# ml-unito/PartitionedLS.jl

Measured on AMD Instinct MI355X. Metric: sign-pattern NNLS solves/sec (whole node); fp64 obj gap vs ref, higher is better.
Workload: dtype f64

## Files before the change

### partitionedls.jl_amd/csrc/opt.hip

```cpp
#include "ctx.h"
#include "near_tie.h"
#include "sweep_rules.h"
#include <algorithm>
#include <chrono>
#include <cmath>
#include <cstdio>
#include <cstring>
#include <functional>
#include <thread>

namespace partls {

static bool opt_range_ok(const partls_ctx *c, const char *who)
{
    if (c->kbits <= 40) return true;
    set_error("%s: %d sign bits: the enumeration of 2^(K+1) patterns is out of range (K <= 39); fit(Alt) and fit(BnB) take up to 61 groups", who, c->kbits);
    return false;
}

static void cleanup_opt(const partls_ctx *c, const std::vector<double> &w, uint64_t pattern, double *alpha, double *beta, double *t)
{
    const int64_t M = c->M, K = c->K;
    std::vector<double> a((size_t)M, 0.0);
    for (int64_t m = 0; m < M; ++m) {
        const int f = sign_of_var(c->mask_aug[(size_t)m], pattern);
        a[(size_t)m] = (f != 0) ? w[(size_t)m] / (double)f : 0.0;
        if (a[(size_t)m] < 0.0) a[(size_t)m] = 0.0;
    }
    std::vector<double> A((size_t)K, 0.0);
    for (int64_t k = 0; k < K; ++k) {
        double s = 0.0;
        for (int64_t m = 0; m < M; ++m) s += (double)c->P[(size_t)m + (size_t)k * M] * a[(size_t)m];
        const double sk = ((pattern >> k) & 1ULL) ? 1.0 : -1.0;
        beta[k] = sk * s;
        A[(size_t)k] = (s == 0.0) ? 1.0 : s;
    }
    for (int64_t m = 0; m < M; ++m) {
        double s = 0.0;
        for (int64_t k = 0; k < K; ++k) s += (double)c->P[(size_t)m + (size_t)k * M] * a[(size_t)m] / A[(size_t)k];
        alpha[m] = s;
    }
    *t = w[(size_t)M];
}

}

using namespace partls;

extern "C" {

partls_status partls_opt_prepare(partls_ctx *c, const double *X, int64_t N, int64_t M, int64_t ldX, const double *y,
                                 int x_on_device, const int64_t *P, int64_t K, int64_t ldP, double eta, uint32_t flags)
try {
    return ctx_prepare(c, X, N, M, ldX, y, x_on_device, P, K, ldP, eta, (flags & PARTLS_OPT_FAITHFUL_INTERCEPT) != 0, flags);
}
PARTLS_ABI_GUARD

partls_status partls_opt_prepare_weighted(partls_ctx *c, const double *X, int64_t N, int64_t M, int64_t ldX, const double *y,
                                          const double *w, int x_on_device, const int64_t *P, int64_t K, int64_t ldP, double eta,
                                          uint32_t flags)
try {
    return ctx_prepare(c, X, N, M, ldX, y, x_on_device, P, K, ldP, eta, (flags & PARTLS_OPT_FAITHFUL_INTERCEPT) != 0, flags, w);
}
PARTLS_ABI_GUARD

partls_status partls_opt_prepare_f32(partls_ctx *c, const float *X, int64_t N, int64_t M, int64_t ldX, const double *y, const double *w,
                                     int x_on_device, const int64_t *P, int64_t K, int64_t ldP, double eta, uint32_t flags)
try {
    return ctx_prepare(c, X, N, M, ldX, y, x_on_device, P, K, ldP, eta, (flags & PARTLS_OPT_FAITHFUL_INTERCEPT) != 0, flags, w, true);
}
PARTLS_ABI_GUARD

partls_status partls_opt_prepare_csr(partls_ctx *c, const int64_t *indptr, const int32_t *indices, const double *values, int64_t N, int64_t M,
                                     const double *y, const double *w, int x_on_device, const int64_t *P, int64_t K, int64_t ldP, double eta,
                                     uint32_t flags)
try {
    return ctx_prepare_csr(c, indptr, indices, values, N, M, y, w, x_on_device, P, K, ldP, eta, (flags & PARTLS_OPT_FAITHFUL_INTERCEPT) != 0, flags);
}
PARTLS_ABI_GUARD

int64_t partls_opt_num_patterns(const partls_ctx *c) { return (c && c->prepared && c->kbits <= 40) ? ((int64_t)1 << c->kbits) : 0; }

static partls_status sweep_second_pass(partls_ctx *c, int64_t g_begin, int64_t g_end, double *all_opt, double *bobj_io, int64_t *bpat_io,
                                       unsigned long long *unconv_io);

partls_status partls_opt_sweep(partls_ctx *c, int64_t g_begin, int64_t g_end, double *best_obj, int64_t *best_pattern,
                               double *all_opt, int64_t *n_unconverged)
try {
    if (!c || !c->prepared) { set_error("partls_opt_sweep: context not prepared"); return PARTLS_ERR_STATE; }
    if (!opt_range_ok(c, "partls_opt_sweep")) return PARTLS_ERR_UNSUPPORTED;
    const int64_t npat = (int64_t)1 << c->kbits;
    if (g_end < 0) g_end = npat;
    if (g_begin < 0 || g_begin > g_end || g_end > npat) { set_error("bad Gray-index range [%lld,%lld)", (long long)g_begin, (long long)g_end); return PARTLS_ERR_BAD_ARG; }
    if (all_opt && !c->faithful) { set_error("all_opt needs PARTLS_OPT_FAITHFUL_INTERCEPT"); return PARTLS_ERR_BAD_ARG; }
    PARTLS_HIP_CHECK(hipSetDevice(c->device));
    if (g_begin == g_end) {
        if (best_obj) *best_obj = INFINITY;
        if (best_pattern) *best_pattern = -1;
        if (n_unconverged) *n_unconverged = 0;
        return PARTLS_OK;
    }
    if (!c->order_ready) {
        partls_status st = prepare_sweep_order(c);
        if (st != PARTLS_OK) return st;
    }
    const int n = c->n;
    const int64_t total = g_end - g_begin;
    int64_t chain_len = 0;
    int grid = 0;
    if (!sweep_plan(c, total, &chain_len, &grid, "partls_opt_sweep")) return PARTLS_ERR_UNSUPPORTED;

    const size_t sweep_words = sweep_block_words(grid, true);
    PARTLS_HIP_CHECK(c->bestObj.ensure(sizeof(double) * sweep_block_words(std::max(grid, 4096), true)));
    PARTLS_HIP_CHECK(hipMemsetAsync(c->bestObj.p, 0, 4 * sizeof(unsigned long long), c->stream));
    if (all_opt) {
        PARTLS_HIP_CHECK(c->allOpt.ensure((size_t)npat * sizeof(double)));
        if (total < npat) PARTLS_HIP_CHECK(hipMemsetAsync(c->allOpt.p, 0xFF, (size_t)npat * sizeof(double), c->stream));
    }
    const partls_status ss = ensure_sweep_scratch(c, grid);
    if (ss != PARTLS_OK) return ss;

    SweepParams p = sweep_params(c, true);
    p.g_begin = g_begin; p.g_end = g_end; p.chain_len = chain_len;
    p.pair = sweep_pairs(c, total) ? 1 : 0;
    p.all_opt = all_opt ? c->allOpt.as<double>() : nullptr;
    bind_sweep_block(p, c->bestObj.as<double>(), grid, true);
    if (!c->use_reg && c->knobs.lz_fault) p.coop_fault = 77;
    c->export_wg = -1;
    if (((c->use_reg && (sweep_reg_small(c->T) || sweep_reg_exports(c->T))) || (!c->use_reg && !c->knobs.eager_generic)) && !c->knobs.no_export) {
        PARTLS_HIP_CHECK(c->bestSol.ensure((size_t)grid * n * sizeof(double)));
        p.best_sol = c->bestSol.as<double>();
        p.node_ld = n;
    }

    t_begin(c, PARTLS_T_SWEEP);
    PARTLS_HIP_CHECK(launch_any_sweep(c, p, grid));
    t_end(c, PARTLS_T_SWEEP);

    unsigned long long cnt[3] = {0, 0, 0};
    PARTLS_HIP_CHECK(c->sweepOut.resize(sweep_words));
    const double *sweep_out = c->sweepOut.data();
    PARTLS_HIP_CHECK(hipMemcpyAsync(c->sweepOut.data(), c->bestObj.p, sweep_words * sizeof(double), hipMemcpyDeviceToHost, c->stream));
    if (all_opt) {
        const void *src = c->allOpt.p;
        if (!c->order_identity) {
            PARTLS_HIP_CHECK(c->allOptRef.ensure((size_t)npat * sizeof(double)));
            PARTLS_HIP_CHECK(launch_pattern_gather(c->allOpt.as<double>(), npat, c->kbits, c->order, c->allOptRef.as<double>(), c->stream));
            src = c->allOptRef.p;
        }
        PARTLS_HIP_CHECK(hipMemcpyAsync(all_opt, src, (size_t)npat * sizeof(double), hipMemcpyDeviceToHost, c->stream));
    }
    PARTLS_HIP_CHECK(hipStreamSynchronize(c->stream));
    t_collect(c);
    std::memcpy(cnt, sweep_out, sizeof(cnt));
    if (c->knobs.print_stamps) {
        double st[32] = {0};
        if (hipMemcpy(st, c->scratch.p, sizeof(st), hipMemcpyDeviceToHost) == hipSuccess)
            fprintf(stderr, "[partls stamps] scan: pre %.0f barrier %.0f post %.0f | gather: work %.0f barrier %.0f | panel: work %.0f barrier %.0f | "
                            "update %.0f | scatter %.0f | chain-load %.0f/%.0f | pivots %llu || gather split: block setup %.0f chain %.0f rhs/myj %.0f"
                            " || workgroup 0: %.0f blocks, %.0f scans, %.0f pivots || pair walk: twin scan %.0f, solve + rows + scan %.0f\n",
                    st[9], st[10], st[0], st[12] + st[13] + st[8], st[1], st[11], st[2], st[3], st[4], st[5], st[6], cnt[1], st[12], st[13], st[8],
                    st[24], st[25], st[26], st[15], st[14]);
    }
    double bobj = INFINITY;
    int64_t bpat = -1;
    install_sweep_result(c, sweep_out, grid, p.best_sol != nullptr, &bobj, &bpat);
    if (rescue_on(c)) {
        rescue_begin_call(c);
        if (cnt[0]) {
            const partls_status rs = sweep_second_pass(c, g_begin, g_end, all_opt, &bobj, &bpat, &cnt[0]);
            if (rs != PARTLS_OK) return rs;
        }
    }
    if (best_obj) *best_obj = bobj;
    if (best_pattern) *best_pattern = bpat;
    if (n_unconverged) *n_unconverged = (int64_t)cnt[0];
    return PARTLS_OK;
}
PARTLS_ABI_GUARD

partls_status partls_opt_finish(partls_ctx *c, int64_t pattern, double *alpha, double *beta, double *t, double *opt,
                                int64_t *best_index)
try {
    if (!c || !c->prepared) { set_error("partls_opt_finish: context not prepared"); return PARTLS_ERR_STATE; }
    if (!alpha || !beta || !t || !opt) { set_error("partls_opt_finish: NULL output"); return PARTLS_ERR_BAD_ARG; }
    if (pattern < 0 || pattern >= ((int64_t)1 << (c->K + 1))) { set_error("pattern out of range"); return PARTLS_ERR_BAD_ARG; }
    PARTLS_HIP_CHECK(hipSetDevice(c->device));
    const uint64_t kmask = ((uint64_t)1 << c->kbits) - 1;
    uint64_t used = 1ULL << c->K;
    for (int i = 0; i < c->n; ++i) if (c->hScale[(size_t)i] != 0.0) used |= c->mask_tab[(size_t)i];

    std::vector<uint64_t> cands{(uint64_t)pattern & kmask & used};
    if (pattern == c->near_for)
        for (int64_t q : c->near_pat) {
            const uint64_t v = (uint64_t)q & kmask & used;
            if (std::find(cands.begin(), cands.end(), v) == cands.end()) cands.push_back(v);
        }
    const int export_wg = (pattern == c->near_for) ? c->export_wg : -1;
    c->export_wg = -1;
    c->near_for = -1;
    c->near_pat.clear();
    c->last_near_evaluated = (int64_t)cands.size();

    t_begin(c, PARTLS_T_FINISH);
    const auto f0 = std::chrono::steady_clock::now();
    std::vector<double> sols, obj2, w, wbest, g, gbest;
    std::vector<int8_t> codes;
    unsigned long long unconv = 0, unconv_best = 0;
    double obest = INFINITY, loo_best = 0.0;
    uint64_t pbest = cands[0];
    for (size_t ci = 0; ci < cands.size(); ++ci) {
        partls_status st = PARTLS_OK;
        bool taken = false;
        if (ci == 0 && export_wg >= 0) {
            PARTLS_HIP_CHECK(c->exportSol.resize((size_t)c->n));
            PARTLS_HIP_CHECK(hipMemcpyAsync(c->exportSol.data(), c->bestSol.as<double>() + (size_t)export_wg * c->n, (size_t)c->n * sizeof(double), hipMemcpyDeviceToHost, c->stream));
            PARTLS_HIP_CHECK(hipStreamSynchronize(c->stream));
            sols.assign(c->exportSol.data(), c->exportSol.data() + c->n);
            opt_codes(c, cands[ci], codes);
            taken = true;
            double smax = 0.0;
            for (int i = 0; i < c->n; ++i) smax = std::max(smax, std::fabs(sols[(size_t)i]));
            for (int i = 0; i < c->n && taken; ++i) {
                const double v = sols[(size_t)i];
                if (!std::isfinite(v)) taken = false;
                else if (v != 0.0 && (codes[(size_t)i] == 0 || (codes[(size_t)i] == 1 && v < -1e-9 * smax) || (codes[(size_t)i] == -1 && v > 1e-9 * smax))) taken = false;
            }
            if (taken) { c->tab_valid = false; unconv = 0; }
            if (c->knobs.finish_trace) fprintf(stderr, "[finish] the sweep's solution of its winner (workgroup %d): %s\n", export_wg, taken ? "taken" : "refused (signs), solving again");
        }
        if (!taken) {
            opt_codes(c, cands[ci], codes);
            st = solve_nodes(c, codes, 1, sols, obj2, &unconv, false, true);
            if (st != PARTLS_OK) return st;
            if (unconv && rescue_on(c)) {
                st = rescue_pattern(c, cands[ci], sols, nullptr, &unconv);
                if (st != PARTLS_OK) return st;
                c->tab_valid = false;
            }
        }
        unscale_solution(c, sols.data(), w);
        RefineOut ro;
        st = refine_solution(c, w, !c->faithful, 2, &ro);
        if (st != PARTLS_OK) return st;
        double o = 0.0;
        if (ro.have) { o = ro.obj; g.swap(ro.g); }
        else { st = data_objective(c, w, &o, &g); if (st != PARTLS_OK) return st; }
        if (c->knobs.finish_trace && cands.size() > 1) fprintf(stderr, "[finish] near tie: pattern %llu data objective %.17g\n", (unsigned long long)cands[ci], o);
        if (ci == 0 || o < obest || (o == obest && cands[ci] < pbest)) { obest = o; pbest = cands[ci]; wbest = w; gbest = g; unconv_best = unconv; loo_best = c->last_min_loo; }
    }
    const auto f1 = std::chrono::steady_clock::now();
    uint64_t full = pbest;
    if (!c->faithful) { if (wbest[(size_t)c->M] > 0.0) full |= (1ULL << c->K); }
    full &= used;
    std::vector<int8_t> vcode((size_t)c->M + 1, 0);
    for (int64_t m = 0; m <= c->M; ++m) {
        if (m == c->M && !c->faithful) { vcode[(size_t)m] = 2; continue; }
        const int f = sign_of_var(c->mask_aug[(size_t)m], full);
        vcode[(size_t)m] = (int8_t)((f > 0) - (f < 0));
    }
    int worst = -1;
    c->last_kkt = kkt_violation_data(c, wbest, gbest, vcode, &worst);
    *opt = obest;
    if (c->knobs.finish_trace) {
        const auto f2 = std::chrono::steady_clock::now();
        auto ms = [](auto a, auto b) { return std::chrono::duration<double, std::milli>(b - a).count(); };
        fprintf(stderr, "[finish] %zu candidate(s): solve + refine + data objective / gradient %.3f ms, KKT check %.3f ms; data-space KKT violation %.3e (variable %d)\n",
                cands.size(), ms(f0, f1), ms(f1, f2), c->last_kkt, worst);
    }
    t_end(c, PARTLS_T_FINISH);
    PARTLS_HIP_CHECK(hipStreamSynchronize(c->stream));
    t_collect(c);
    cleanup_opt(c, wbest, full, alpha, beta, t);
    if (best_index) *best_index = (int64_t)full;
    if (unconv_best) { set_error("winner re-solve hit the pivot cap"); return PARTLS_ERR_NOT_CONVERGED; }
    c->last_min_loo = loo_best;
    if (kkt_says_ill_conditioned(c)) {
        set_error("the winner's KKT conditions do not hold in data space (violation %.2e of ||x|| ||y|| at variable %d, tolerance %.1e; %llu columns "
                  "refused as dependent in the sweep): X is too ill-conditioned for the fp64 Gram form (cond(X) >~ 1e6); the outputs hold the best "
                  "Gram-form model", c->last_kkt, worst, c->knobs.kkt_tol, c->sweep_vetoes);
        return PARTLS_ERR_ILL_CONDITIONED;
    }
    return PARTLS_OK;
}
PARTLS_ABI_GUARD

partls_status partls_opt_pattern(partls_ctx *c, int64_t pattern, double *raw_alpha, double *optval)
try {
    if (!c || !c->prepared) { set_error("partls_opt_pattern: context not prepared"); return PARTLS_ERR_STATE; }
    if (!c->faithful) { set_error("partls_opt_pattern needs a context prepared with PARTLS_OPT_FAITHFUL_INTERCEPT"); return PARTLS_ERR_STATE; }
    if (pattern < 0 || pattern >= ((int64_t)1 << c->kbits)) { set_error("pattern out of range"); return PARTLS_ERR_BAD_ARG; }
    PARTLS_HIP_CHECK(hipSetDevice(c->device));
    std::vector<double> sols, obj2, w;
    unsigned long long unconv = 0;
    std::vector<int8_t> codes;
    opt_codes(c, (uint64_t)pattern, codes);
    partls_status st = solve_nodes(c, codes, 1, sols, obj2, &unconv, false, true);
    if (st != PARTLS_OK) return st;
    if (unconv && rescue_on(c)) {
        st = rescue_pattern(c, (uint64_t)pattern, sols, nullptr, &unconv);
        if (st != PARTLS_OK) return st;
        c->tab_valid = false;
    }
    unscale_solution(c, sols.data(), w);
    st = refine_solution(c, w, false);
    if (st != PARTLS_OK) return st;
    if (optval) { st = data_objective(c, w, optval); if (st != PARTLS_OK) return st; }
    if (raw_alpha)
        for (int64_t m = 0; m <= c->M; ++m) {
            const int f = sign_of_var(c->mask_aug[(size_t)m], (uint64_t)pattern);
            const double a = (f != 0) ? w[(size_t)m] / (double)f : 0.0;
            raw_alpha[m] = a > 0.0 ? a : 0.0;
        }
    if (unconv) { set_error("pattern solve hit the pivot cap"); return PARTLS_ERR_NOT_CONVERGED; }
    return PARTLS_OK;
// ... 437 lines not shown
```

### partitionedls.jl_amd/csrc/sweep_blk.hip

```cpp
#include "sweep_rules.h"
#include <atomic>
#include <type_traits>

namespace partls {
namespace blk {

static constexpr int THREADS = 512;
static constexpr int MAXT = 20;
#ifndef PARTLS_UPD_UNROLL
#define PARTLS_UPD_UNROLL 1
#endif
static constexpr int MB = 8;
#ifndef PARTLS_EXPORT_BIG
#define PARTLS_EXPORT_BIG 1
#endif
#ifndef PARTLS_MERGED_SCAN
#define PARTLS_MERGED_SCAN 1
#endif
#ifndef PARTLS_LANE_MASKS
#define PARTLS_LANE_MASKS 1
#endif
#ifndef PARTLS_MB_BIG
#define PARTLS_MB_BIG 8
#endif
#ifndef PARTLS_PAIR
#define PARTLS_PAIR 1
#endif
static constexpr int EXPORT_MAXT = 17;
static constexpr int MBB = PARTLS_MB_BIG;
static constexpr int NO_VETO = 99;
static constexpr int PAIR_MAXC = 16;
static constexpr int PAIR_PIV_MIN_HI = 0x3f1a36e2;
static constexpr int F64_EXP_HI = 0x7ff00000;

constexpr int nslots(int T) { return T * (T + 1) / 2; }
constexpr int tri(int g) { return g * (g + 1) / 2; }
constexpr int split(int T)
{
    int best = 1, bestmax = 1 << 30;
    for (int g = 1; g < T; ++g) {
        int a = tri(g), b = nslots(T) - tri(g);
        int m = a > b ? a : b;
        if (m < bestmax) { bestmax = m; best = g; }
    }
    return T == 1 ? 1 : best;
}
constexpr int rstride(int T) { return (T % 2) ? T : T + 1; }
constexpr int colw(int T) { return 513; }
static constexpr int MAXT_S = 10;
static constexpr int CW_S = 257;
template <class PT> __device__ __forceinline__ PT *uniform_ptr(PT *p)
{
    const unsigned long long v = (unsigned long long)p;
    const unsigned lo = (unsigned)__builtin_amdgcn_readfirstlane((int)v), hi = (unsigned)__builtin_amdgcn_readfirstlane((int)(v >> 32));
    return (PT *)(((unsigned long long)hi << 32) | lo);
}

#ifdef PARTLS_STAMPS
#define STAMP_DECL unsigned long long st_acc[24] = {0, 0, 0, 0, 0, 0, 0, 0, 0, 0, 0, 0, 0, 0, 0, 0, 0, 0, 0, 0, 0, 0, 0, 0}; unsigned long long st_t = __builtin_amdgcn_s_memtime();
#define STAMP(ph) do { __builtin_amdgcn_sched_barrier(0); unsigned long long _n = __builtin_amdgcn_s_memtime(); \
                       st_acc[ph] += _n - st_t; st_t = _n; __builtin_amdgcn_sched_barrier(0); } while (0)
#ifndef PARTLS_STAMP_TID
#define PARTLS_STAMP_TID 0
#endif
#define STAMP_FLUSH do { if (tid == PARTLS_STAMP_TID && blockIdx.x == 0 && p.scratch) { for (int _i = 0; _i < 24; ++_i) p.scratch[_i] = (double)st_acc[_i]; \
                                p.scratch[24] = (double)bc; p.scratch[25] = (double)sc; p.scratch[26] = (double)npiv; } } while (0)
#else
#define STAMP_DECL
#define STAMP(ph) do { } while (0)
#define STAMP_FLUSH do { } while (0)
#endif

static constexpr int CWMAX = colw(MAXT);
template <int CWX, int MAXTX>
struct LdsImageT {
    double Z[MB * CWX];
    double U[2 * (MB + 64)];
    double Dinv[MB + 64];
    unsigned long long s_inf[32];
    unsigned long long s_bas[16];
    unsigned long long s_sum[16];
    int s_veto[2];
    double s_best[4];
    unsigned char s_rbit[64];
    unsigned long long s_vmask[16 * MAXTX];
    double Pbase[2 * MB * CWX];
};
struct LdsImage {
    double Z[MBB * CWMAX];
    double U[2 * (MBB + 64)];
    double Dinv[MBB + 64];
    unsigned long long s_inf[32];
    unsigned long long s_bas[16];
    unsigned long long s_sum[16];
    int s_veto[2];
    double s_best[4];
    unsigned char s_rbit[64];
    unsigned long long s_vmask[16 * MAXT];
    double Pbase[2 * MBB * CWMAX];
};
static_assert(2 * MBB >= PAIR_MAXC, "the pair walk gathers up to PAIR_MAXC columns into the two panel buffers");
__shared__ LdsImage lds_image;
__shared__ LdsImageT<CW_S, MAXT_S> lds_small;

template <int W>
__device__ __forceinline__ auto *image_of()
{
    if constexpr (W == 1) return &lds_small; else return &lds_image;
}

template <int T, int H, int W = 2>
struct Half {
    static constexpr int G = W == 1 ? T : split(T);
    static constexpr int GLO = H ? G : 0;
    static constexpr int GHI = H ? T : G;
    static constexpr int OFF = H ? tri(G) : 0;
    static constexpr int CNT = (H ? nslots(T) - tri(G) : tri(G)) > 0 ? (H ? nslots(T) - tri(G) : tri(G)) : 1;
    static constexpr int XN = GHI;
    static constexpr int RS = rstride(T);
    static constexpr int CW = W == 1 ? CW_S : colw(T);
    static constexpr int NT = W == 1 ? 256 : THREADS;
    __device__ static constexpr int idx(int rho, int gam) { return tri(gam) + rho - OFF; }
};

template <class L>
__device__ __forceinline__ void tiles_store(double *dst, const double (&S)[L::CNT], int t8)
{
    double *bp = uniform_ptr(dst) + (size_t)L::OFF * 256;
#pragma unroll
    for (int s = 0; s < L::CNT; ++s) {
        if ((s & 1) == 0) asm volatile("" : "+s"(bp));
        bp[(s & 1) * 256 + t8] = S[s];
        if (s & 1) bp += 512;
    }
}

template <int T, int H, int W, int KAPPA, class SA>
__device__ __forceinline__ void gather_tile(const SA &S, double *P, int a, int b, unsigned pm)
{
    using L = Half<T, H, W>;
    if constexpr (KAPPA >= L::GLO && KAPPA < L::GHI) {
        if ((pm >> b) & 1u) {
            double *col = P + __builtin_popcount(pm & ((1u << b) - 1u)) * L::CW + a * L::RS;
#pragma unroll
            for (int rho = 0; rho <= KAPPA; ++rho) col[rho] = S[L::idx(rho, KAPPA)];
        }
    }
    if ((pm >> a) & 1u) {
        double *col = P + __builtin_popcount(pm & ((1u << a) - 1u)) * L::CW + b * L::RS;
#pragma unroll
        for (int gam = (KAPPA + 1 > L::GLO ? KAPPA + 1 : L::GLO); gam < L::GHI; ++gam) col[gam] = S[L::idx(KAPPA, gam)];
    }
}

template <int T, int H, int W, int KAPPA, class SA>
__device__ __forceinline__ void scatter_tile(SA &S, const double *P, int a, int b, unsigned pm)
{
    using L = Half<T, H, W>;
    if constexpr (KAPPA >= L::GLO && KAPPA < L::GHI) {
        if ((pm >> b) & 1u) {
            const double *col = P + __builtin_popcount(pm & ((1u << b) - 1u)) * L::CW + a * L::RS;
#pragma unroll
            for (int rho = 0; rho <= KAPPA; ++rho) S[L::idx(rho, KAPPA)] = col[rho];
        }
    }
    if ((pm >> a) & 1u) {
        const double *col = P + __builtin_popcount(pm & ((1u << a) - 1u)) * L::CW + b * L::RS;
#pragma unroll
        for (int gam = (KAPPA > L::GLO ? KAPPA : L::GLO); gam < L::GHI; ++gam) S[L::idx(KAPPA, gam)] = col[gam];
    }
}

template <int M, int CW, int MBK>
__device__ __forceinline__ int panel_block(double *P, double *Z, double *U, double *Dinv, int myj, bool my_basic,
                                           double piv_eps, int tid, int prow, bool idle_wave)
{
    if (idle_wave) {
#pragma unroll
        for (int s = 0; s < M; ++s) __syncthreads();
        return M;
    }
    constexpr int US = MBK + 64;
    const int dummy = MBK + (tid & 63);
    double pv[M];
#pragma unroll
    for (int j = 0; j < M; ++j) pv[j] = P[j * CW + prow];
    const int uslot = myj >= 0 ? myj : dummy;
    int veto = M;
#pragma unroll
    for (int s = 0; s < M; ++s) {
        Z[s * CW + prow] = pv[s];
        U[(s & 1) * US + uslot] = pv[s];
        if (myj == s) {
            const double d = pv[s];
            Dinv[s] = (my_basic || d > piv_eps) ? rcp_newton(d) : 0.0;
        }
        __syncthreads();
        double inv = Dinv[s];
        double u[M];
#pragma unroll
        for (int j = 0; j < M; ++j) u[j] = U[(s & 1) * US + j];
        asm volatile("" : "+v"(inv));
#pragma unroll
        for (int j = 0; j < M; ++j) asm volatile("" : "+v"(u[j]));
        if ((pv[s] * pv[s]) * (inv * piv_eps) >= 1.0) veto = veto < s ? veto : s;
        if (__builtin_amdgcn_readfirstlane(__double2hiint(inv)) & 0x7ff00000) {
            const double ainv = fabs(inv), fz = -pv[s] * inv;
            if (myj == s) {
#pragma unroll
                for (int j = 0; j < M; ++j) pv[j] = (j == s) ? -inv : u[j] * ainv;
            } else {
#pragma unroll
                for (int j = 0; j < M; ++j) pv[j] = (j == s) ? pv[s] * ainv : fma(fz, u[j], pv[j]);
            }
        }
    }
#pragma unroll
    for (int j = 0; j < M; ++j) P[j * CW + prow] = pv[j];
    return veto;
}

template <int CW, int RS, int KC>
__device__ __forceinline__ void pair_solve(const double *P, const int *cpos, int m, int lane, int rhspos, double *out)
{
    const int r = lane & 15, h = lane >> 4;
    const int code = cpos[r < m ? r : 0];
    const unsigned basm = (unsigned)__ballot(code < 0 && lane < m);
    const int kr = code < 0 ? ~code : code;
    const int pos = kr * RS + KC;
    double pv[4];
#pragma unroll
    for (int jj = 0; jj < 4; ++jj) {
        const int c = 4 * h + jj;
        const int cc = cpos[c < m ? c : 0];
        const double v = P[(cc < 0 ? ~cc : cc) * CW + pos];
        pv[jj] = (r < m && c < m) ? v : 0.0;
    }
    double qc = P[kr * CW + rhspos];
    if (r >= m) qc = 0.0;
    bool hard = false;
#pragma unroll 1
    for (int s = 0; s < m; ++s) {
        const double d = readlane_f64(pv[0], s);
        const int dh = __double2hiint(d);
        if ((!((basm >> s) & 1u) && !(dh > PAIR_PIV_MIN_HI)) || (dh & F64_EXP_HI) == F64_EXP_HI) { hard = true; break; }
        const double inv = rcp_newton(d), ainv = fabs(inv);
        const double pvs = __shfl(pv[0], r);
        const double fz = -pvs * inv;
        const double qs = readlane_f64(qc, s);
        double val[4];
#pragma unroll
        for (int jj = 0; jj < 4; ++jj) {
            const double u = __shfl(pv[0], (s + 4 * h + jj) & 15);
            val[jj] = (r == s) ? u * ainv : fma(fz, u, pv[jj]);
        }
        if (h == 0) val[0] = (r == s) ? -inv : pvs * ainv;
        qc = (r == s) ? qs * ainv : fma(fz, qs, qc);
        const double nx = __shfl(val[0], (lane + 16) & 63);
        pv[0] = val[1]; pv[1] = val[2]; pv[2] = val[3]; pv[3] = nx;
    }
    if (lane < PAIR_MAXC) {
        out[PAIR_MAXC + lane] = qc;
        out[lane] = ((basm >> lane) & 1u) ? -qc : qc;
    }
    if (lane == 0) out[2 * PAIR_MAXC + 1] = hard ? 1.0 : 0.0;
}

#define PARTLS_CASES(M) M(0) M(1) M(2) M(3) M(4) M(5) M(6) M(7) M(8) M(9) M(10) M(11) M(12) M(13) M(14) M(15) M(16) M(17) M(18) M(19)

template <int T, int H, bool NODE, int W = 2, bool MODELS = false, bool BATCH = false, bool PAIRK = false>
__device__ __forceinline__ void sweep_body(const SweepParams &p)
{
    using L = Half<T, H, W>;
    constexpr int RS = L::RS, CW = L::CW, RHSPOS = 16 * RS, NW = (T + 3) / 4;
    constexpr int THREADS = L::NT;
    constexpr int MB = W == 1 ? blk::MB : MBB;
    static_assert(!(NODE && MODELS), "node mode exports no per-pattern models (finish_pattern's capped flag is chain mode's)");
    constexpr bool MERGED = PARTLS_MERGED_SCAN && !NODE && !BATCH && T <= 17;
    constexpr bool LANE_MASKS = PARTLS_LANE_MASKS && !BATCH && T <= 16;
    constexpr bool PAIR = PAIRK && PARTLS_PAIR && MERGED && LANE_MASKS && W == 2 && !MODELS;
    static_assert(PAIR == PAIRK, "the pair walk is launched only where it is compiled (pair_compiled)");
    static_assert(W == 2 || RHSPOS < 256, "the 256-thread kernel needs every panel row position (and the rhs row) below 256");
    auto &lds_image = *image_of<W>();
    const int tid = threadIdx.x, t8 = tid & 255, a = t8 & 15, b = t8 >> 4, lane = tid & 63, wave = tid >> 6;
    const int n = p.n;
    const int nwords = (n + 63) >> 6;

    double *const Pbase = lds_image.Pbase, *const Z = lds_image.Z, *const U = lds_image.U, *const Dinv = lds_image.Dinv;
    unsigned long long *const s_inf = lds_image.s_inf, *const s_bas = lds_image.s_bas, *const s_vmask = lds_image.s_vmask;
    unsigned long long *const s_sum = lds_image.s_sum;
    int *const s_veto = lds_image.s_veto;
    double *const s_best = lds_image.s_best;
    [[maybe_unused]] double *const s_pair = U;
    [[maybe_unused]] int *const s_cpos = reinterpret_cast<int *>(Dinv);
    [[maybe_unused]] int *const s_tw = s_cpos + PAIR_MAXC;
    [[maybe_unused]] int *const s_cm = s_tw + 8;
    static_assert(2 * (MB + 64) >= 2 * PAIR_MAXC + 2, "pair_solve's `out` (doubles) fits U");
    static_assert(2 * (MB + 64) >= PAIR_MAXC + 9, "s_cpos, s_tw and s_cm (PAIR_MAXC + 9 ints) fit Dinv (MB + 64 doubles)");
    for (int i = tid; i < 2 * MB * CW; i += THREADS) Pbase[i] = 0.0;
    for (int i = tid; i < MB * CW; i += THREADS) Z[i] = 0.0;
    if (tid < 2 * (MB + 64)) U[tid] = 0.0;
    if (tid < MB + 64) Dinv[tid] = 0.0;
    if (tid < 32) s_inf[tid] = 0;
    if (tid < 16) { s_bas[tid] = 0; s_sum[tid] = 0; }
    if (tid < 2) s_veto[tid] = NO_VETO;
    if (tid == 0) {
        s_best[0] = __builtin_inf(); reinterpret_cast<long long *>(s_best)[1] = -1;
        s_best[2] = __builtin_inf(); reinterpret_cast<long long *>(s_best)[3] = -1;
    }
    if (tid < 16 * T) s_vmask[tid] = tid < p.n ? p.mask[tid] : 0ULL;
    if (tid < 64) lds_image.s_rbit[tid] = tid < 40 ? p.rbit.gbit[tid] : 0;
    __syncthreads();

    double S[L::CNT];
    double q = 0.0, corner = 0.0;
    double mybest = __builtin_inf();
    const bool has_var = tid < n;
    bool basic = false, blocked = false;
    const int mypos = (tid & 15) * RS + (tid >> 4);
    const int rowc = tid / RS, rowrho = tid - rowc * RS;
    const bool idle_wave = __builtin_amdgcn_readfirstlane((tid & ~63) > RHSPOS ? 1 : 0) != 0;

    unsigned npiv = 0, nunconv = 0, nveto = 0;
    unsigned bc = 0, sc = 0;

    const int clen = (int)p.chain_len;
    const int nchains = (int)((p.g_end - p.g_begin + clen - 1) / clen);

    STAMP_DECL
    for (int chain = blockIdx.x; chain < nchains; chain += gridDim.x) {
        const int64_t g0 = p.g_begin + (int64_t)chain * clen;
        const int glen = (int)((g0 + clen < p.g_end) ? clen : p.g_end - g0);
        STAMP(5);
        const double *src = p.T0;
        if constexpr (NODE) {
            if (p.node_src) {
                const double *snap = p.node_src[chain];
                if (snap) src = snap;
            }
        }
        {
            const double *bp = uniform_ptr(src) + (size_t)L::OFF * 256;
#pragma unroll
            for (int s = 0; s < L::CNT; ++s) {
                if ((s & 1) == 0) asm volatile("" : "+s"(bp));
                S[s] = bp[(s & 1) * 256 + t8];
                if (s & 1) bp += 512;
            }
        }
        q = (tid < 16 * T) ? src[(size_t)nslots(T) * 256 + tid] : 0.0;
        corner = src[(size_t)nslots(T) * 256 + 16 * T];
        basic = false;
        if constexpr (NODE) {
            if (src != p.T0 && tid < 16 * T) basic = reinterpret_cast<const int8_t *>(src + (nslots(T) * 256 + 16 * T + 8))[tid] != 0;
        }
        STAMP(6);

        auto finish_pattern = [&](int gi, [[maybe_unused]] bool capped) {
            const uint64_t g = (uint64_t)g0 + (unsigned)gi;
            const uint64_t pat = NODE ? (uint64_t)chain : g ^ (g >> 1);
            const double obj2 = corner > 0.0 ? corner : 0.0;
            if constexpr (NODE) {
                if (p.node_piv && tid == 0) {
                    unsigned *o = p.node_piv + 3 * ((size_t)chain * clen + gi);
                    o[0] = npiv; o[1] = bc; o[2] = sc;
                }
            }
            if (p.all_opt && tid == THREADS - 1) p.all_opt[pat] = sqrt(obj2);
            if constexpr (MODELS) {
                const size_t row = (size_t)chain * (size_t)clen + (size_t)gi;
                if (has_var) p.node_sol[row * p.node_ld + tid] = capped ? __builtin_nan("") : (basic ? q : 0.0);
                if (tid == THREADS - 1) p.node_obj2[row] = capped ? __builtin_nan("") : sqrt(obj2);
            }
            if constexpr (!NODE && !MODELS && (W == 1 || (PARTLS_EXPORT_BIG && T <= EXPORT_MAXT))) {
                if (p.best_sol && obj2 < mybest) {
                    mybest = obj2;
                    if (has_var) p.best_sol[(size_t)blockIdx.x * p.node_ld + tid] = basic ? q : 0.0;
                }
            }
            if (tid == THREADS - 1 && obj2 <= s_best[2]) {
                const double bo = s_best[0];
                const long long bp = reinterpret_cast<long long *>(s_best)[1];
                if (obj2 < bo || (obj2 == bo && ref_index_less(pat, (unsigned long long)bp, lds_image.s_rbit))) {
                    s_best[2] = bo; reinterpret_cast<long long *>(s_best)[3] = bp;
                    s_best[0] = obj2; reinterpret_cast<long long *>(s_best)[1] = (long long)pat;
                } else if (obj2 < s_best[2] || ref_index_less(pat, (unsigned long long)reinterpret_cast<long long *>(s_best)[3], lds_image.s_rbit)) {
                    s_best[2] = obj2; reinterpret_cast<long long *>(s_best)[3] = (long long)pat;
                }
            }
        };
        [[maybe_unused]] auto record_twin = [&](int gi, double cornerv, double qv, bool bv) {
            const uint64_t g = (uint64_t)g0 + (unsigned)gi;
            const uint64_t pat = g ^ (g >> 1);
            const double obj2 = cornerv > 0.0 ? cornerv : 0.0;
            if (p.all_opt && tid == THREADS - 1) p.all_opt[pat] = sqrt(obj2);
            if constexpr (PARTLS_EXPORT_BIG && T <= EXPORT_MAXT) {
                if (p.best_sol && obj2 < mybest) {
                    mybest = obj2;
                    if (has_var) p.best_sol[(size_t)blockIdx.x * p.node_ld + tid] = bv ? qv : 0.0;
                }
            }
            if (tid == THREADS - 1 && obj2 <= s_best[2]) {
                const double bo = s_best[0];
                const long long bp = reinterpret_cast<long long *>(s_best)[1];
                if (obj2 < bo || (obj2 == bo && ref_index_less(pat, (unsigned long long)bp, lds_image.s_rbit))) {
                    s_best[2] = bo; reinterpret_cast<long long *>(s_best)[3] = bp;
                    s_best[0] = obj2; reinterpret_cast<long long *>(s_best)[1] = (long long)pat;
                } else if (obj2 < s_best[2] || ref_index_less(pat, (unsigned long long)reinterpret_cast<long long *>(s_best)[3], lds_image.s_rbit)) {
                    s_best[2] = obj2; reinterpret_cast<long long *>(s_best)[3] = (long long)pat;
                }
            }
        };
        int gi = 0;
        [[maybe_unused]] bool tw_pending = false;
        [[maybe_unused]] auto pair_partner = [&](int i) -> int {
            const int j = (((unsigned)g0 + (unsigned)i) & 1u) ? i - 1 : i + 1;
            return (PAIR && j >= 0 && j < glen) ? j : -1;
        };
        [[maybe_unused]] auto pair_unit_end = [&](int i) -> int { const int j = pair_partner(i); return (j > i ? j : i) + 1; };
        [[maybe_unused]] auto pair_target = [&](int u, int i) -> int {
            const unsigned gu = (unsigned)g0 + (unsigned)u, gc = (unsigned)g0 + (unsigned)i;
            if (pair_partner(u) < 0 || (gu & 1u)) return u;
            return (((gu >> 1) ^ gu ^ (gc >> 1) ^ gc) & 1u) ? u + 1 : u;
        };
        [[maybe_unused]] auto pair_next = [&](bool to_twin, int &f, int &fn) -> bool {
            if (to_twin) gi = pair_partner(gi);
            else {
                const int u = pair_unit_end(gi);
                if (u >= glen) return false;
                gi = pair_target(u, gi);
            }
            tw_pending = !to_twin && pair_partner(gi) >= 0;
            const uint64_t vmask = s_vmask[tid < 16 * T ? tid : 0] & (has_var ? ~0ULL : 0ULL);
            const uint64_t g = (uint64_t)g0 + (unsigned)gi;
            f = sign_of_var(vmask, g ^ (g >> 1));
            const int u2 = pair_unit_end(gi);
            fn = f;
            if (u2 < glen) { const uint64_t gn = (uint64_t)g0 + (unsigned)pair_target(u2, gi); fn = sign_of_var(vmask, gn ^ (gn >> 1)); }
            return true;
        };
        for (;;) {
            [[maybe_unused]] const unsigned nunconv0 = nunconv;
            bool isfree = false;
            int f = 0;
            [[maybe_unused]] int fn = 0;
            if constexpr (NODE) {
                const int code = has_var ? (int)p.node_code[((size_t)chain * clen + gi) * p.node_ld + tid] : 0;
                isfree = code == 2;
                f = isfree ? 0 : code;
            } else {
                const uint64_t vmask = s_vmask[tid < 16 * T ? tid : 0] & (has_var ? ~0ULL : 0ULL);
                const uint64_t g = (uint64_t)g0 + (unsigned)gi, gn = g + 1;
                f = sign_of_var(vmask, g ^ (g >> 1));
                if constexpr (MERGED) fn = glen > 1 ? sign_of_var(vmask, gn ^ (gn >> 1)) : f;
                if constexpr (PAIR) {
                    tw_pending = pair_partner(0) >= 0;
                    const int u2 = pair_unit_end(0);
                    fn = f;
                    if (u2 < glen) { const uint64_t g2 = (uint64_t)g0 + (unsigned)pair_target(u2, 0); fn = sign_of_var(vmask, g2 ^ (g2 >> 1)); }
                }
            }
            blocked = false;
            int ninf_best = n + 1, patience = 3, rounds = 0;
            bool progress = false;
            for (;;) {
                if (progress) blocked = false;
                progress = false;
                const int par = sc & 1;
                ++sc;
                bool bad = false;
                [[maybe_unused]] bool nxt = false;
                if (has_var) {
                    const double fq = q * (double)(f > 1 ? 1 : (f < -1 ? -1 : f));
                    if (NODE && isfree) bad = !basic && !blocked && (fabs(q) > p.tol);
                    else if (basic) bad = (f == 0) || (fq < -p.tol);
                    else bad = (fq > p.tol) && !blocked;
                    if constexpr (MERGED) {
                        const double fqn = q * (double)(fn > 1 ? 1 : (fn < -1 ? -1 : fn));
                        nxt = basic ? ((fn == 0) || (fqn < -p.tol)) : (fqn > p.tol);
                    }
                }
                const unsigned long long bb = __ballot(bad), bs = __ballot(basic);
                unsigned summ = (unsigned)__popcll(bb);
#pragma unroll
                for (int sub = 0; sub < 4; ++sub)
                    if ((bb >> (16 * sub)) & 0xFFFFull) summ |= 0x100u << sub;
                if constexpr (!MERGED) {
                    if (lane == 0 && wave < nwords) { s_inf[par * 8 + wave] = bb; s_bas[par * 8 + wave] = bs; s_sum[par * 8 + wave] = summ; }
                } else {
                    const unsigned long long bn = __ballot(nxt);
                    unsigned summ2 = (unsigned)__popcll(bn);
#pragma unroll
                    for (int sub = 0; sub < 4; ++sub)
                        if ((bn >> (16 * sub)) & 0xFFFFull) summ2 |= 0x100u << sub;
                    if (lane == 0 && wave < nwords) {
                        s_inf[par * 8 + wave] = bb; s_inf[16 + par * 8 + wave] = bn; s_bas[par * 8 + wave] = bs;
                        s_sum[par * 8 + wave] = ((unsigned long long)summ2 << 32) | summ;
                    }
                }
                STAMP(9);
                __syncthreads();
                STAMP(10);
                int count = 0;
                unsigned tiles = 0;
                [[maybe_unused]] int count2 = 0;
                [[maybe_unused]] unsigned tiles2 = 0;
#pragma unroll
                for (int w = 0; w < NW; ++w) {
                    const unsigned long long sw2 = s_sum[par * 8 + w];
                    const unsigned sw = (unsigned)__builtin_amdgcn_readfirstlane((int)sw2);
                    count += (int)(sw & 0xFFu);
                    tiles |= (sw >> 8) << (4 * w);
                    if constexpr (MERGED) {
                        const unsigned sn = (unsigned)__builtin_amdgcn_readfirstlane((int)(sw2 >> 32));
                        count2 += (int)(sn & 0xFFu);
                        tiles2 |= (sn >> 8) << (4 * w);
                    }
                }
                STAMP(0);
                int soff = par * 8;
                bool all = true;
                bool done = count == 0;
                if (!done) {
                    if (count < ninf_best) { ninf_best = count; patience = 3; }
                    else if (patience > 0) --patience;
                    else all = false;
                    if (++rounds > p.max_rounds) { ++nunconv; done = true; }
                }
                if (done) {
                    if constexpr (!MERGED) break;
                    finish_pattern(gi, count != 0);
                    if constexpr (PAIR) {
                        int tw = 0;
                        if (tw_pending) {
                            tw = 2;
                            if (count == 0) {
                                constexpr int KC = T - 2, WQ = (16 * KC) >> 6, SHQ = (16 * KC) & 63;
                                static_assert(KC >= L::G, "the pair column's tile slots all lie in half 1");
                                int tidp = tid;
                                asm volatile("" : "+v"(tidp));
                                const int lanep = tidp & 63, wavep = __builtin_amdgcn_readfirstlane(tidp >> 6), kp = tidp & 15;
                                const bool mine = (tidp >> 4) == KC;
                                const uint64_t vmask = s_vmask[tidp < 16 * T ? tidp : 0] & (has_var ? ~0ULL : 0ULL);
                                const uint64_t gt = (uint64_t)g0 + (unsigned)pair_partner(gi);
                                const int ft = sign_of_var(vmask, gt ^ (gt >> 1));
                                gather_tile<T, H, W, KC>(S, Pbase, a, b, 0xFFFFu);
                                if (mine) Pbase[kp * CW + RHSPOS] = q;
                                if (H == 0 && wavep == WQ) {
                                    const double fqt = q * (double)(ft > 1 ? 1 : (ft < -1 ? -1 : ft));
                                    const bool badt = mine && has_var && (basic ? ((ft == 0) || (fqt < -p.tol)) : (fqt > p.tol));
                                    const unsigned cmw = (unsigned)(__ballot(badt) >> SHQ) & 0xFFFFu;
                                    if (badt) s_cpos[__builtin_popcount(cmw & ((1u << kp) - 1u))] = basic ? ~kp : kp;
                                    if (lanep == 0) s_cm[0] = (int)cmw;
                                }
                                __syncthreads();
                                STAMP(15);
                                const unsigned cm = (unsigned)__builtin_amdgcn_readfirstlane(s_cm[0]);
                                if (cm == 0) {
                                    record_twin(pair_partner(gi), corner, q, basic);
                                    tw = 0;
                                } else {
                                    if (H == 0 && wavep == 3) pair_solve<CW, RS, KC>(Pbase, s_cpos, __builtin_popcount(cm), lanep, RHSPOS, s_pair);
                                    __syncthreads();
                                    const bool guard = __builtin_amdgcn_readfirstlane(__double2hiint(s_pair[2 * PAIR_MAXC + 1])) != 0;
                                    const bool in_c = mine && ((cm >> kp) & 1u);
                                    double qt = q, cornert = corner;
                                    {
                                        const int rp = tidp < 16 * T ? kp * RS + (tidp >> 4) : RHSPOS;
                                        int j = 0;
                                        for (unsigned mm = cm; mm; mm &= mm - 1u, ++j) {
                                            const int k = __builtin_ctz(mm);
                                            const double aj = s_pair[j];
                                            qt = fma(-Pbase[k * CW + rp], aj, qt);
                                            cornert = fma(-Pbase[k * CW + RHSPOS], aj, cornert);
                                        }
                                    }
                                    if (in_c) qt = s_pair[PAIR_MAXC + __builtin_popcount(cm & ((1u << kp) - 1u))];
                                    const bool bt = basic != in_c;
                                    const double fqt = qt * (double)(ft > 1 ? 1 : (ft < -1 ? -1 : ft));
                                    const bool bad2 = has_var && (bt ? ((ft == 0) || (fqt < -p.tol)) : (fqt > p.tol));
                                    const unsigned long long b2 = __ballot(bad2);
                                    if (lanep == 0) s_tw[wavep] = b2 != 0ull;
                                    __syncthreads();
                                    int left = guard ? 1 : 0;
#pragma unroll
                                    for (int w = 0; w < 8; ++w) left |= s_tw[w];
                                    left = __builtin_amdgcn_readfirstlane(left);
                                    if (!left) { record_twin(pair_partner(gi), cornert, qt, bt); tw = 0; }
                                }
                                STAMP(14);
                            }
                        }
                        if (tw == 2) {
                            if (!pair_next(true, f, fn)) break;
                            blocked = false;
                            ninf_best = n + 1; patience = 3; rounds = 0;
                            continue;
                        }
                    }
                    {
                    if constexpr (PAIR) { if (!pair_next(false, f, fn)) break; }
                    else if (++gi >= glen) break;
                    blocked = false;
                    ninf_best = n + 1; patience = 3; rounds = 0;
                    if constexpr (MERGED) {
                        if constexpr (!PAIR) {
                        const uint64_t vmask = s_vmask[tid < 16 * T ? tid : 0] & (has_var ? ~0ULL : 0ULL);
                        const uint64_t gn = (uint64_t)g0 + (unsigned)gi + 1;
                        f = fn;
                        fn = gi + 1 < glen ? sign_of_var(vmask, gn ^ (gn >> 1)) : f;
                        }
                        if (count2 == 0 || p.max_rounds < 1) continue;
                        ninf_best = count2; rounds = 1;
                        all = true;
                        tiles = tiles2;
                        soff += 16;
                    }
                    }
                }
                int single_k = -1;
                if (!all) {
#pragma unroll
                    for (int w = 0; w < NW; ++w) {
                        unsigned long long ww = s_inf[par * 8 + w];
                        ww = ((unsigned long long)(unsigned)__builtin_amdgcn_readfirstlane((int)(ww >> 32)) << 32) |
                             (unsigned)__builtin_amdgcn_readfirstlane((int)ww);
                        if (ww) single_k = (w << 6) + 63 - __builtin_clzll(ww);
                    }
                    tiles = 1u << (single_k >> 4);
                }
                tiles = (unsigned)__builtin_amdgcn_readfirstlane((int)tiles);
                [[maybe_unused]] unsigned tmask = 0;
                if constexpr (LANE_MASKS) {
                    const int tl = lane < T ? lane : 0, wl = tl >> 2, shl = 16 * (tl & 3);
                    tmask = (unsigned)((s_inf[soff + wl] >> shl) & 0xFFFFull) | ((unsigned)((s_bas[par * 8 + wl] >> shl) & 0xFFFFull) << 16);
                }

                while (tiles) {
                    const int kappa = __builtin_ctz(tiles);
                    unsigned pmall, basm;
                    if constexpr (LANE_MASKS) {
                        const unsigned tm = (unsigned)__builtin_amdgcn_readlane((int)tmask, kappa);
                        pmall = tm & 0xFFFFu;
                        if (!all) pmall = 1u << (single_k & 15);
                        basm = tm >> 16;
                    } else {
                        const int wsel = kappa >> 2, sh = 16 * (kappa & 3);
                        pmall = (unsigned)((s_inf[soff + wsel] >> sh) & 0xFFFFull);
                        if (!all) pmall = 1u << (single_k & 15);
                        basm = (unsigned)__builtin_amdgcn_readfirstlane((int)((s_bas[par * 8 + wsel] >> sh) & 0xFFFFull));
                        pmall = (unsigned)__builtin_amdgcn_readfirstlane((int)pmall);
                    }
                    while (pmall) {
                        unsigned rest = 0;
                        if (__builtin_expect(__builtin_popcount(pmall) > MB, 0)) {
                            rest = pmall;
#pragma unroll
                            for (int i = 0; i < MB; ++i) rest &= rest - 1;
                        }
                        const unsigned pm = pmall & ~rest;
                        pmall = rest;
                        const int m = __builtin_popcount(pm);
                        const int bpar = bc & 1;
                        double *P = Pbase + bpar * MB * CW;
                        ++bc;
                        int kap = kappa;
                        asm volatile("" : "+s"(kap));
                        STAMP(12);
#define PARTLS_G(i) if constexpr (i < T) { if (__builtin_expect(kap == i, 0)) gather_tile<T, H, W, i>(S, P, a, b, pm); }
                        PARTLS_CASES(PARTLS_G)
#undef PARTLS_G
                        STAMP(13);
                        if (tid < 16 * T && (tid >> 4) == kappa && ((pm >> (tid & 15)) & 1u))
                            P[__builtin_popcount(pm & ((1u << (tid & 15)) - 1u)) * CW + RHSPOS] = q;
                        int myj = -1;
                        bool my_basic = false;
                        if (rowrho == kappa && rowc < 16 && ((pm >> rowc) & 1u)) {
                            myj = __builtin_popcount(pm & ((1u << rowc) - 1u));
                            my_basic = (basm >> rowc) & 1u;
                        }
                        STAMP(8);
                        __syncthreads();
                        STAMP(1);
                        if (tid == 0) s_veto[bpar ^ 1] = NO_VETO;
                        {
                            int veto;
                            switch (m) {
#define PARTLS_PB(i) case i: if constexpr (i <= MB) veto = panel_block<(i <= MB ? i : 1), CW, MB>(P, Z, U, Dinv, myj, my_basic, p.piv_eps, tid, tid, idle_wave); else veto = 0; break;
                                PARTLS_PB(1) PARTLS_PB(2) PARTLS_PB(3) PARTLS_PB(4) PARTLS_PB(5) PARTLS_PB(6) PARTLS_PB(7) PARTLS_PB(8)
                                PARTLS_PB(9) PARTLS_PB(10) PARTLS_PB(11) PARTLS_PB(12) PARTLS_PB(13) PARTLS_PB(14) PARTLS_PB(15)
#undef PARTLS_PB
                                default: veto = panel_block<MB, CW, MB>(P, Z, U, Dinv, myj, my_basic, p.piv_eps, tid, tid, idle_wave); break;
                            }
                            if (veto < m && tid != RHSPOS) atomicMin(&s_veto[bpar], veto);
                        }
                        STAMP(11);
                        __syncthreads();
                        STAMP(2);
                        const int vs = __builtin_amdgcn_readfirstlane(s_veto[bpar]);
                        unsigned pmx = pm;
                        int mx = m;
                        if (__builtin_expect(vs < m, 0)) {
                            unsigned r = pm;
                            for (int i = 0; i < vs; ++i) r &= r - 1;
                            const unsigned vbit = r & (0u - r);
                            blocked = blocked || (tid == 16 * kappa + __builtin_ctz(vbit));
                            pmall |= pm & ~vbit;
                            pmx = 0;
                            mx = 0;
                            ++nveto;
                        }
                        bool blk_ok = false;
#pragma unroll PARTLS_UPD_UNROLL
                        for (int s = 0; s < mx; ++s) {
                            const double inv = Dinv[s];
                            blk_ok = blk_ok || (inv != 0.0);
                            const double *Zs = Z + s * CW;
                            double x[L::XN];
#pragma unroll
                            for (int rho = 0; rho < L::XN; ++rho) x[rho] = Zs[a * RS + rho];
#pragma unroll
                            for (int gam = L::GLO; gam < L::GHI; ++gam) {
                                const double yg = -Zs[b * RS + gam] * inv;
#pragma unroll
                                for (int rho = 0; rho <= gam; ++rho)
                                    S[L::idx(rho, gam)] = fma(x[rho], yg, S[L::idx(rho, gam)]);
                            }
                            const double zr = Zs[RHSPOS], zri = zr * inv;
                            if (tid < 16 * T) q = fma(-Zs[mypos], zri, q);
                            corner = fma(-zr, zri, corner);
                        }
                        STAMP(3);
#define PARTLS_F(i) if constexpr (i < T) { if (__builtin_expect(kap == i, 0)) scatter_tile<T, H, W, i>(S, P, a, b, pmx); }
                        PARTLS_CASES(PARTLS_F)
#undef PARTLS_F
                        if (tid < 16 * T && (tid >> 4) == kappa && ((pmx >> (tid & 15)) & 1u)) {
                            const int j = __builtin_popcount(pmx & ((1u << (tid & 15)) - 1u));
                            q = P[j * CW + RHSPOS];
                            if (Dinv[j] != 0.0) basic = !basic;
                            else blocked = true;
                        }
                        progress = progress || blk_ok;
                        npiv += (unsigned)mx;
// ... 200 lines not shown
```

Before: 24.92 million.

## Index pair solve by fixed 16-column tile with masks instead of compacted positions

The pair-walk solve no longer compacts violating columns into an LDS position list. It works on the full 16-wide tile column, using a candidate bitmask and a basic-variable bitmask packed into one shared word, and skips columns outside the mask. The row update after the solve now runs as an unrolled DPP broadcast-FMA sequence over all 16 columns instead of a variable-length loop over set bits. This removes LDS index indirection and data-dependent loops, but does fixed 16-column work even when few columns are active, and it relies on hand-written inline assembly with hazard nops. Extra stamp phases are added for profiling.

Result: faster. 26.32 million (median of 6 runs) (+5.6%).

```diff
diff --git a/partitionedls.jl_amd/csrc/opt.hip b/partitionedls.jl_amd/csrc/opt.hip
--- a/partitionedls.jl_amd/csrc/opt.hip
+++ b/partitionedls.jl_amd/csrc/opt.hip
@@ -158,9 +158,11 @@
         if (hipMemcpy(st, c->scratch.p, sizeof(st), hipMemcpyDeviceToHost) == hipSuccess)
             fprintf(stderr, "[partls stamps] scan: pre %.0f barrier %.0f post %.0f | gather: work %.0f barrier %.0f | panel: work %.0f barrier %.0f | "
                             "update %.0f | scatter %.0f | chain-load %.0f/%.0f | pivots %llu || gather split: block setup %.0f chain %.0f rhs/myj %.0f"
-                            " || workgroup 0: %.0f blocks, %.0f scans, %.0f pivots || pair walk: twin scan %.0f, solve + rows + scan %.0f\n",
+                            " || workgroup 0: %.0f blocks, %.0f scans, %.0f pivots || pair walk: twin scan %.0f, solve + rows + scan %.0f"
+                            " = solve prologue %.0f steps %.0f (both on the solving wave only: PARTLS_STAMP_TID=192) barrier behind the solve %.0f"
+                            " rows %.0f verdict %.0f\n",
                     st[9], st[10], st[0], st[12] + st[13] + st[8], st[1], st[11], st[2], st[3], st[4], st[5], st[6], cnt[1], st[12], st[13], st[8],
-                    st[24], st[25], st[26], st[15], st[14]);
+                    st[24], st[25], st[26], st[15], st[16] + st[17] + st[18] + st[19] + st[20], st[16], st[17], st[18], st[19], st[20]);
     }
     double bobj = INFINITY;
     int64_t bpat = -1;
diff --git a/partitionedls.jl_amd/csrc/sweep_blk.hip b/partitionedls.jl_amd/csrc/sweep_blk.hip
--- a/partitionedls.jl_amd/csrc/sweep_blk.hip
+++ b/partitionedls.jl_amd/csrc/sweep_blk.hip
@@ -65,10 +65,14 @@
 #endif
 #define STAMP_FLUSH do { if (tid == PARTLS_STAMP_TID && blockIdx.x == 0 && p.scratch) { for (int _i = 0; _i < 24; ++_i) p.scratch[_i] = (double)st_acc[_i]; \
                                 p.scratch[24] = (double)bc; p.scratch[25] = (double)sc; p.scratch[26] = (double)npiv; } } while (0)
+#define STAMP_PARAMS , unsigned long long (&st_acc)[24], unsigned long long &st_t
+#define STAMP_ARGS , st_acc, st_t
 #else
 #define STAMP_DECL
 #define STAMP(ph) do { } while (0)
 #define STAMP_FLUSH do { } while (0)
+#define STAMP_PARAMS
+#define STAMP_ARGS
 #endif
 
 static constexpr int CWMAX = colw(MAXT);
@@ -221,47 +225,45 @@
 }
 
 template <int CW, int RS, int KC>
-__device__ __forceinline__ void pair_solve(const double *P, const int *cpos, int m, int lane, int rhspos, double *out)
+__device__ __forceinline__ void pair_solve(const double *P, unsigned cm, unsigned basm, int lane, int rhspos, double *out STAMP_PARAMS)
 {
     const int r = lane & 15, h = lane >> 4;
-    const int code = cpos[r < m ? r : 0];
-    const unsigned basm = (unsigned)__ballot(code < 0 && lane < m);
-    const int kr = code < 0 ? ~code : code;
-    const int pos = kr * RS + KC;
+    const int pos = r * RS + KC;
     double pv[4];
 #pragma unroll
-    for (int jj = 0; jj < 4; ++jj) {
-        const int c = 4 * h + jj;
-        const int cc = cpos[c < m ? c : 0];
-        const double v = P[(cc < 0 ? ~cc : cc) * CW + pos];
-        pv[jj] = (r < m && c < m) ? v : 0.0;
-    }
-    double qc = P[kr * CW + rhspos];
-    if (r >= m) qc = 0.0;
+    for (int jj = 0; jj < 4; ++jj) pv[jj] = P[(4 * h + jj) * CW + pos];
+    double qc = P[r * CW + rhspos];
     bool hard = false;
+    STAMP(16);
 #pragma unroll 1
-    for (int s = 0; s < m; ++s) {
-        const double d = readlane_f64(pv[0], s);
-        const int dh = __double2hiint(d);
-        if ((!((basm >> s) & 1u) && !(dh > PAIR_PIV_MIN_HI)) || (dh & F64_EXP_HI) == F64_EXP_HI) { hard = true; break; }
-        const double inv = rcp_newton(d), ainv = fabs(inv);
-        const double pvs = __shfl(pv[0], r);
-        const double fz = -pvs * inv;
-        const double qs = readlane_f64(qc, s);
-        double val[4];
+    for (int hq = 0; hq < 4 && !hard; ++hq) {
 #pragma unroll
         for (int jj = 0; jj < 4; ++jj) {
-            const double u = __shfl(pv[0], (s + 4 * h + jj) & 15);
-            val[jj] = (r == s) ? u * ainv : fma(fz, u, pv[jj]);
+            const int s = 4 * hq + jj;
+            if (hard || !((cm >> s) & 1u)) continue;
+            const double d = readlane_f64(pv[jj], 16 * hq + s);
+            const int dh = __double2hiint(d);
+            if ((!((basm >> s) & 1u) && !(dh > PAIR_PIV_MIN_HI)) || (dh & F64_EXP_HI) == F64_EXP_HI) { hard = true; continue; }
+            const double inv = rcp_newton(d), ainv = fabs(inv);
+            const double pvs = __shfl(pv[jj], 16 * hq + r);
+            const double fz = -pvs * inv;
+            const double qs = readlane_f64(qc, s);
+            double u[4];
+#pragma unroll
+            for (int j2 = 0; j2 < 4; ++j2) u[j2] = __shfl(pv[jj], 16 * hq + 4 * h + j2);
+#pragma unroll
+            for (int j2 = 0; j2 < 4; ++j2) {
+                const double v = (r == s) ? u[j2] * ainv : fma(fz, u[j2], pv[j2]);
+                pv[j2] = (j2 == jj && h == hq) ? ((r == s) ? -inv : pvs * ainv) : v;
+            }
+            qc = (r == s) ? qs * ainv : fma(fz, qs, qc);
         }
-        if (h == 0) val[0] = (r == s) ? -inv : pvs * ainv;
-        qc = (r == s) ? qs * ainv : fma(fz, qs, qc);
-        const double nx = __shfl(val[0], (lane + 16) & 63);
-        pv[0] = val[1]; pv[1] = val[2]; pv[2] = val[3]; pv[3] = nx;
-    }
+    }
+    STAMP(17);
     if (lane < PAIR_MAXC) {
+        const bool in_c = (cm >> lane) & 1u;
         out[PAIR_MAXC + lane] = qc;
-        out[lane] = ((basm >> lane) & 1u) ? -qc : qc;
+        out[lane] = in_c ? (((basm >> lane) & 1u) ? -qc : qc) : 0.0;
     }
     if (lane == 0) out[2 * PAIR_MAXC + 1] = hard ? 1.0 : 0.0;
 }
@@ -292,11 +294,11 @@
     int *const s_veto = lds_image.s_veto;
     double *const s_best = lds_image.s_best;
     [[maybe_unused]] double *const s_pair = U;
-    [[maybe_unused]] int *const s_cpos = reinterpret_cast<int *>(Dinv);
-    [[maybe_unused]] int *const s_tw = s_cpos + PAIR_MAXC;
+    [[maybe_unused]] int *const s_tw = reinterpret_cast<int *>(Dinv);
     [[maybe_unused]] int *const s_cm = s_tw + 8;
+    static_assert(PAIR_MAXC == 16, "the pair column is one tile column: 16 variables, one mask bit each");
     static_assert(2 * (MB + 64) >= 2 * PAIR_MAXC + 2, "pair_solve's `out` (doubles) fits U");
-    static_assert(2 * (MB + 64) >= PAIR_MAXC + 9, "s_cpos, s_tw and s_cm (PAIR_MAXC + 9 ints) fit Dinv (MB + 64 doubles)");
+    static_assert(2 * (MB + 64) >= 9, "s_tw and s_cm (9 ints) fit Dinv (MB + 64 doubles)");
     for (int i = tid; i < 2 * MB * CW; i += THREADS) Pbase[i] = 0.0;
     for (int i = tid; i < MB * CW; i += THREADS) Z[i] = 0.0;
     if (tid < 2 * (MB + 64)) U[tid] = 0.0;
@@ -550,32 +552,44 @@
                                     const double fqt = q * (double)(ft > 1 ? 1 : (ft < -1 ? -1 : ft));
                                     const bool badt = mine && has_var && (basic ? ((ft == 0) || (fqt < -p.tol)) : (fqt > p.tol));
                                     const unsigned cmw = (unsigned)(__ballot(badt) >> SHQ) & 0xFFFFu;
-                                    if (badt) s_cpos[__builtin_popcount(cmw & ((1u << kp) - 1u))] = basic ? ~kp : kp;
-                                    if (lanep == 0) s_cm[0] = (int)cmw;
+                                    const unsigned basw = (unsigned)(__ballot(basic) >> SHQ) & 0xFFFFu;
+                                    if (lanep == 0) s_cm[0] = (int)(cmw | (basw << 16));
                                 }
                                 __syncthreads();
                                 STAMP(15);
-                                const unsigned cm = (unsigned)__builtin_amdgcn_readfirstlane(s_cm[0]);
+                                const unsigned cmb = (unsigned)__builtin_amdgcn_readfirstlane(s_cm[0]);
+                                const unsigned cm = cmb & 0xFFFFu;
                                 if (cm == 0) {
                                     record_twin(pair_partner(gi), corner, q, basic);
                                     tw = 0;
                                 } else {
-                                    if (H == 0 && wavep == 3) pair_solve<CW, RS, KC>(Pbase, s_cpos, __builtin_popcount(cm), lanep, RHSPOS, s_pair);
+                                    if (H == 0 && wavep == 3) pair_solve<CW, RS, KC>(Pbase, cm, cmb >> 16, lanep, RHSPOS, s_pair STAMP_ARGS);
+                                    else STAMP(16);
                                     __syncthreads();
+                                    STAMP(18);
                                     const bool guard = __builtin_amdgcn_readfirstlane(__double2hiint(s_pair[2 * PAIR_MAXC + 1])) != 0;
                                     const bool in_c = mine && ((cm >> kp) & 1u);
                                     double qt = q, cornert = corner;
                                     {
-                                        const int rp = tidp < 16 * T ? kp * RS + (tidp >> 4) : RHSPOS;
-                                        int j = 0;
-                                        for (unsigned mm = cm; mm; mm &= mm - 1u, ++j) {
-                                            const int k = __builtin_ctz(mm);
-                                            const double aj = s_pair[j];
-                                            qt = fma(-Pbase[k * CW + rp], aj, qt);
-                                            cornert = fma(-Pbase[k * CW + RHSPOS], aj, cornert);
-                                        }
+                                        const double *prow = Pbase + (tidp < 16 * T ? kp * RS + (tidp >> 4) : RHSPOS);
+                                        const double na = -s_pair[kp], qk = Pbase[kp * CW + RHSPOS];
+                                        double tq;
+#define PARTLS_ROW(K, PAD) asm volatile("s_nop " #PAD "\n\t" \
+                                          "v_mov_b64_dpp %2, %4 row_newbcast:" #K " row_mask:0xf bank_mask:0xf\n\t" \
+                                          "v_fmac_f64_dpp %0, %3, %5 row_newbcast:" #K " row_mask:0xf bank_mask:0xf\n\t" \
+                                          "s_nop 0\n\t" \
+                                          "v_fmac_f64_dpp %1, %3, %2 row_newbcast:" #K " row_mask:0xf bank_mask:0xf" \
+                                          : "+v"(qt), "+v"(cornert), "=&v"(tq) : "v"(na), "v"(qk), "v"(pk[K]));
+                                        double pk[PAIR_MAXC];
+#pragma unroll
+                                        for (int k = 0; k < PAIR_MAXC; ++k) pk[k] = prow[k * CW];
+                                        PARTLS_ROW(0, 4) PARTLS_ROW(1, 1) PARTLS_ROW(2, 1) PARTLS_ROW(3, 1) PARTLS_ROW(4, 1) PARTLS_ROW(5, 1)
+                                        PARTLS_ROW(6, 1) PARTLS_ROW(7, 1) PARTLS_ROW(8, 1) PARTLS_ROW(9, 1) PARTLS_ROW(10, 1) PARTLS_ROW(11, 1)
+                                        PARTLS_ROW(12, 1) PARTLS_ROW(13, 1) PARTLS_ROW(14, 1) PARTLS_ROW(15, 1)
+#undef PARTLS_ROW
                                     }
-                                    if (in_c) qt = s_pair[PAIR_MAXC + __builtin_popcount(cm & ((1u << kp) - 1u))];
+                                    if (in_c) qt = s_pair[PAIR_MAXC + kp];
+                                    STAMP(19);
                                     const bool bt = basic != in_c;
                                     const double fqt = qt * (double)(ft > 1 ? 1 : (ft < -1 ? -1 : ft));
                                     const bool bad2 = has_var && (bt ? ((ft == 0) || (fqt < -p.tol)) : (fqt > p.tol));
@@ -588,7 +602,7 @@
                                     left = __builtin_amdgcn_readfirstlane(left);
                                     if (!left) { record_twin(pair_partner(gi), cornert, qt, bt); tw = 0; }
                                 }
-                                STAMP(14);
+                                STAMP(20);
                             }
                         }
                         if (tw == 2) {
```
